# NGoetz/NF

Measured on NVIDIA B200. Metric: nis_flow_fwd_logdet_points_per_sec, higher is better.
Workload: dtype f32

## Files before the change

### nf_b200/csrc/flow_tc_h.cu

```cuda
#include <stdlib.h>
#include <cuda_fp16.h>
#include "common.cuh"
#include "spline.cuh"
#include "flow_fwd_common.cuh"
#include "tc_common.cuh"
#include "tc_spline.cuh"

#define H_SA 8.0f
#define H_AMAX 65504.0f
#define H_HID_BYTES (2 * TCH * TCH * 2)
#define H_MAXG 4
template <int KIND> struct HK {
    static constexpr int OUT_N = KIND == NIS_KIND_PWLIN ? 64 : 80;
    static constexpr int TPER = KIND == NIS_KIND_PWLIN ? 2 : 1;
    static constexpr int SLOT = KIND == NIS_KIND_PWLIN ? 32 : 80;
    static constexpr int COLS = KIND == NIS_KIND_PWLIN ? 128 : 160;
    static constexpr int COL_AHI = KIND == NIS_KIND_PWLIN ? 64 : 96;
    static constexpr int COL_ALO = COL_AHI + 32;
    static constexpr int MAXG = KIND == NIS_KIND_PWLIN ? 4 : 3;
};
__host__ __device__ static inline int h_slot(const DevFlow& F) { return F.kind == NIS_KIND_PWLIN ? 32 : 80; }
__host__ __device__ static inline int h_out_rows(const DevFlow& F) {
    int mt = 1;
    for (int c = 0; c < F.n_cells; ++c) mt = F.cells[c].T > mt ? F.cells[c].T : mt;
    const int r = mt * h_slot(F);
    return F.kind == NIS_KIND_PWLIN ? (r < 128 ? 128 : r) : r;
}
__host__ __device__ static inline int h_out_bytes(const DevFlow& F) { return 2 * h_out_rows(F) * TCH * 2; }

__host__ __device__ static inline int h_off(int row, int k) {
    return (row >> 3) * 1024 + (row & 7) * 128 + ((((k >> 3) ^ (row & 7)) << 4) | ((k & 7) << 1));
}
__host__ __device__ constexpr uint32_t h_idesc(int M, int N) {
    return (1u << 4) | ((uint32_t)(N >> 3) << 17) | ((uint32_t)(M >> 4) << 24);
}
__host__ __device__ static inline size_t h_l0_off(const DevFlow& F) { return (size_t)(F.depth - 1) * H_HID_BYTES + h_out_bytes(F); }
__host__ __device__ static inline size_t h_cell_bytes(const DevFlow& F) { return h_l0_off(F) + H_HID_BYTES + 64; }

__device__ __forceinline__ float ex2_approx(float x) {
    float y;
    asm("ex2.approx.ftz.f32 %0, %1;" : "=f"(y) : "f"(x));
    return y;
}

__device__ __forceinline__ uint32_t h_pack_sat(float x, float y) {
    uint32_t d;
    asm("cvt.rn.satfinite.f16x2.f32 %0, %1, %2;" : "=r"(d) : "f"(y), "f"(x));
    return d;
}

__device__ __forceinline__ void h_mma_ts(uint32_t tmem_d, uint32_t tmem_a, uint64_t desc_b, uint32_t idesc, uint32_t accumulate) {
    asm volatile(
        "{\n\t.reg .pred p;\n\tsetp.ne.b32 p, %4, 0;\n\t"
        "tcgen05.mma.cta_group::1.kind::f16 [%0], [%1], %2, %3, p;\n\t}"
        ::"r"(tmem_d), "r"(tmem_a), "l"(desc_b), "r"(idesc), "r"(accumulate) : "memory");
}

__global__ void __launch_bounds__(256) flow_h_pack_kernel(DevFlow F, const float* __restrict__ params, char* __restrict__ hpack) {
    __shared__ float red[8];
    __shared__ float sw_s;
    const int c = blockIdx.y, li = blockIdx.x, tid = threadIdx.x;
    const DevCell& q = F.cells[c];
    const bool outl = li == F.depth - 1, first = li == F.depth;
    const int l = first ? 0 : li + 1;
    const float* w = params + q.param_off + F.p_lin(c, l);
    const int kin = first ? q.P : TCH;
    const int rows_src = outl ? q.T * F.K : TCH, rows = outl ? h_out_rows(F) : TCH, slot = h_slot(F);
    float m = 0.f;
    for (int i = tid; i < rows_src * kin; i += 256) m = fmaxf(m, fabsf(w[i]));
#pragma unroll
    for (int o = 16; o > 0; o >>= 1) m = fmaxf(m, __shfl_xor_sync(0xffffffffu, m, o));
    if ((tid & 31) == 0) red[tid >> 5] = m;
    __syncthreads();
    if (tid == 0) {
        for (int i = 1; i < 8; ++i) m = fmaxf(m, red[i]);
        int e = 14;
        if (m > 0.f && m < 3.0e38f) frexpf(m, &e);
        e = e < -100 ? -100 : (e > 100 ? 100 : e);
        sw_s = ldexpf(1.f, 14 - e);
    }
    __syncthreads();
    const float SW = sw_s;
    char* dst = hpack + (size_t)c * h_cell_bytes(F);
    char* hi = dst + (first ? h_l0_off(F) : (size_t)li * H_HID_BYTES);
    char* lo = hi + (size_t)rows * TCH * 2;
    for (int i = tid; i < rows * TCH; i += 256) {
        const int n = i / TCH, k = i - n * TCH;
        const int t = outl ? n / slot : 0, jj = outl ? n - t * slot : n;
        const bool live = outl ? (t < q.T && jj < F.K) : k < kin;
        const float v = live ? w[(size_t)(outl ? t * F.K + jj : n) * kin + k] * SW : 0.f;
        const __half h = __float2half_rn(v);
        const int o = h_off(n, k);
        *reinterpret_cast<__half*>(hi + o) = h;
        *reinterpret_cast<__half*>(lo + o) = __float2half_rn(v - __half2float(h));
    }
    if (tid == 0) reinterpret_cast<float*>(dst + h_cell_bytes(F) - 64)[l] = 1.f / (H_SA * SW);
}

struct HSmem {
    int w0, aff, bias, st, sst, red, zb, total;
    int wfirst;
    __host__ __device__ int wl(int l) const { return (l - wfirst) * H_HID_BYTES; }
};
__host__ __device__ static inline HSmem h_layout(const DevFlow& F, int P, int l_begin, int l_end, bool zstage, int NG,
                                                 bool layer0 = true, bool stats = true) {
    HSmem s;
    int o = 0;
    s.wfirst = l_begin > 1 ? l_begin : 1;
    for (int l = s.wfirst; l <= l_end; ++l) o += l == F.depth ? h_out_bytes(F) : H_HID_BYTES;
    (void)P;
    s.w0 = o; o += layer0 ? H_HID_BYTES : 0;
    s.aff = o; o += (F.depth + 1) * 2 * TCH * 4;
    s.bias = o; o += h_out_rows(F) * 4;
    s.st = o; o += NG * (F.d + 1) * TCM * 4;
    o = (o + 15) & ~15;
    s.sst = o; o += NG * (F.d + 1) * TCM * 4;
    o = (o + 7) & ~7;
    s.red = o; o += stats ? (NG * TCM * 2 + 2 * F.maxW) * 8 : 0;
    o = (o + 127) & ~127;
    s.zb = o;
    if (zstage) o += NG * TCH * TCM * 4;
    s.total = o;
    return s;
}

__device__ __forceinline__ void h_store_act32(const float* v, const float* sc, const float* sh, uint32_t t_hi, uint32_t t_lo) {
    uint32_t hi[16], lo[16];
#pragma unroll
    for (int j4 = 0; j4 < 8; ++j4) {
        const float4 s4 = reinterpret_cast<const float4*>(sc)[j4], h4 = reinterpret_cast<const float4*>(sh)[j4];
        const float a0 = fmaxf(fmaf(v[4 * j4], s4.x, h4.x), 0.f), a1 = fmaxf(fmaf(v[4 * j4 + 1], s4.y, h4.y), 0.f);
        const float a2 = fmaxf(fmaf(v[4 * j4 + 2], s4.z, h4.z), 0.f), a3 = fmaxf(fmaf(v[4 * j4 + 3], s4.w, h4.w), 0.f);
        const uint32_t p01 = h_pack_sat(a0, a1), p23 = h_pack_sat(a2, a3);
        const float2 f01 = __half22float2(*reinterpret_cast<const __half2*>(&p01));
        const float2 f23 = __half22float2(*reinterpret_cast<const __half2*>(&p23));
        hi[2 * j4] = p01;
        hi[2 * j4 + 1] = p23;
        lo[2 * j4] = h_pack_sat(a0 - f01.x, a1 - f01.y);
        lo[2 * j4 + 1] = h_pack_sat(a2 - f23.x, a3 - f23.y);
    }
    tc_st16(t_hi, hi);
    tc_st16(t_lo, lo);
}

__device__ __forceinline__ void h_issue_block(uint32_t tmem_d, uint32_t t_hi, uint32_t t_lo, uint32_t w_hi, uint32_t w_lo, uint32_t idesc) {
#pragma unroll
    for (int ks = 0; ks < 4; ++ks) {
        h_mma_ts(tmem_d, t_hi + ks * 8, tc_desc(w_lo + ks * 32), idesc, ks > 0);
        h_mma_ts(tmem_d, t_lo + ks * 8, tc_desc(w_hi + ks * 32), idesc, 1);
    }
#pragma unroll
    for (int ks = 0; ks < 4; ++ks) h_mma_ts(tmem_d, t_hi + ks * 8, tc_desc(w_hi + ks * 32), idesc, 1);
}

template <int NG, int KIND, int MODE>
__global__ void __launch_bounds__(NG * TCM, 1) flow_cell_h_kernel(const __grid_constant__ DevFlow F, const FwdArgs A,
                                                                        const char* __restrict__ hpack) {
    constexpr int NT = NG * TCM;
    typedef HK<KIND> K_;
    constexpr int H_COLS = K_::COLS, H_COL_AHI = K_::COL_AHI, H_COL_ALO = K_::COL_ALO;
    extern __shared__ char smraw[];
    __shared__ uint64_t a_ready[NG], d_ready[NG], z_full[NG], s_full[NG];
    __shared__ uint32_t tmem_base_s;
    char* sm = smem_align1024(smraw);
    const int tid = threadIdx.x, warp = tid >> 5, lane = tid & 31;
    const int c = A.c_begin;
    const DevCell& q = F.cells[c];
    const int d = F.d, depth = F.depth;
    constexpr bool stats = (MODE & 1) != 0;
    constexpr bool from_z = (MODE & 2) != 0;
    constexpr bool nextmom = (MODE & 4) != 0;
    constexpr bool needs_state = !(from_z && stats);
    constexpr int MOM_N = 4 + 4 * 5 / 2;
    float macc[nextmom ? MOM_N : 1];
#pragma unroll
    for (int i = 0; i < (nextmom ? MOM_N : 1); ++i) macc[i] = 0.f;
    const int lz = from_z ? (A.zin_layer > 0 ? A.zin_layer : (stats ? A.stats_layer - 1 : depth)) : 1;
    const int l_end = stats ? A.stats_layer - 1 : depth;
    const bool zst = from_z || stats;
    const HSmem L = h_layout(F, q.P, lz, l_end, zst, NG, !from_z, stats);
    float* affs = reinterpret_cast<float*>(sm + L.aff);
    float* biass = reinterpret_cast<float*>(sm + L.bias);
    const float* pk = A.wpack + q.pk_off;
    const char* cellpack = hpack + (size_t)c * h_cell_bytes(F);
    const float* inv_scale = reinterpret_cast<const float*>(cellpack + h_cell_bytes(F) - 64);

    for (int l = L.wfirst; l <= l_end; ++l) {
        const int n16 = (l == depth ? h_out_bytes(F) : H_HID_BYTES) / 16;
        const uint4* src = reinterpret_cast<const uint4*>(cellpack + (size_t)(l - 1) * H_HID_BYTES);
        uint4* dst = reinterpret_cast<uint4*>(sm + L.wl(l));
        for (int i = tid; i < n16; i += NT) dst[i] = src[i];
    }
    if (!from_z) {
        const uint4* src = reinterpret_cast<const uint4*>(cellpack + h_l0_off(F));
        uint4* dst = reinterpret_cast<uint4*>(sm + L.w0);
        for (int i = tid; i < H_HID_BYTES / 16; i += NT) dst[i] = src[i];
    }
    for (int l = 0; l <= depth; ++l) {
        const int W = l == 0 ? q.P : TCH, Wp = pad8(W);
        const float* s = pk + q.aff_off[l];
        const float f = H_SA;
        const float fs = (l >= 1 && l >= lz && l <= l_end) ? f * inv_scale[l - 1] : f;
        for (int i = tid; i < W; i += NT) { affs[l * 2 * TCH + i] = fs * s[i]; affs[l * 2 * TCH + TCH + i] = f * s[Wp + i]; }
    }
    const int out_rows = h_out_rows(F);
    constexpr float LOGIT_UNIT = 1.4426950408889634f;
    for (int i = tid; i < out_rows; i += NT) {
        const int t = i / K_::SLOT, jj = i - t * K_::SLOT;
        biass[i] = (t < q.T && jj < F.K) ? LOGIT_UNIT * pk[q.bo_off + t * F.Kpad + jj] : 0.f;
    }
    if (tid == 0) {
        for (int g = 0; g < NG; ++g) {
            mbar_init(&a_ready[g], TCM); mbar_init(&d_ready[g], 1); mbar_init(&z_full[g], 1); mbar_init(&s_full[g], 1);
        }
        asm volatile("fence.mbarrier_init.release.cluster;" ::: "memory");
    }
    if (warp == 0) {
        asm volatile("tcgen05.alloc.cta_group::1.sync.aligned.shared::cta.b32 [%0], %1;" ::"r"(smem_u32(&tmem_base_s)), "r"(512));
        asm volatile("tcgen05.relinquish_alloc_permit.cta_group::1.sync.aligned;" ::);
    }
    proxy_fence();
    tc_fence_before();
    __syncthreads();
    tc_fence_after();
    const uint32_t tmem_base = tmem_base_s;
    const long long ntiles = (A.B + TCM - 1) / TCM;
    const long long rowlen = d + 1;
    const int nblk = (q.T + K_::TPER - 1) / K_::TPER;
    const bool has_out = l_end == depth;
    double dsum = 0.0, dsq = 0.0;

    const uint32_t idesc = h_idesc(TCM, TCH), idesc_out = h_idesc(TCM, K_::OUT_N);
    {
        const int g = warp >> 2, gt = tid & (TCM - 1);
        float* st = reinterpret_cast<float*>(sm + L.st) + g * (d + 1) * TCM + gt;
        const uint32_t tg = tmem_base + g * H_COLS + ((uint32_t)((warp & 3) * 32) << 16);
        uint32_t pd = 0, pa = 0, zph = 0, sph = 0;
        float* zs = reinterpret_cast<float*>(sm + L.zb) + g * TCH * TCM;
        constexpr uint32_t ZBYTES = TCH * TCM * 4;
        float* sst = reinterpret_cast<float*>(sm + L.sst) + g * (d + 1) * TCM;
        const uint32_t SBYTES = (uint32_t)((d + 1) * TCM * 4);
        const bool st_bulk = needs_state && A.from_state && (reinterpret_cast<uintptr_t>(A.state_in) & 15) == 0 && (SBYTES & 15) == 0;
        if (st_bulk && gt == 0) {
            const long long t0 = (long long)blockIdx.x * NG + g;
            if ((t0 + 1) * TCM <= A.B) bulk_load(sst, A.state_in + t0 * TCM * rowlen, SBYTES, &s_full[g]);
        }
        const float inv_out = has_out ? LOGIT_UNIT * inv_scale[depth] : 0.f;
        for (long long it = 0;; ++it) {
            const long long tile = ((long long)blockIdx.x + it * gridDim.x) * NG + g;
            if (tile >= ntiles) break;
            const long long tn = tile + (long long)gridDim.x * NG;
            if (from_z && gt == 0) {
                if (A.zout) bulk_store_wait_read();
                bulk_load(zs, A.zin + (size_t)tile * TCH * TCM, ZBYTES, &z_full[g]);
                if (tn < ntiles) bulk_prefetch_l2(A.zin + (size_t)tn * TCH * TCM, ZBYTES);
            }
            const long long pt = tile * TCM + gt;
            const bool valid = pt < A.B;
            if (!needs_state) {
            } else if (st_bulk && (tile + 1) * TCM <= A.B) {
                mbar_wait(&s_full[g], sph);
                sph ^= 1;
                for (int i = 0; i <= d; ++i) st[i * TCM] = sst[gt * rowlen + i];
                proxy_fence();
                group_sync(g);
                if (gt == 0 && (tn + 1) * TCM <= A.B) bulk_load(sst, A.state_in + tn * TCM * rowlen, SBYTES, &s_full[g]);
            } else if (valid) {
                if (A.from_state) {
                    for (int i = 0; i <= d; ++i) st[i * TCM] = A.state_in[pt * rowlen + i];
                } else {
                    for (int i = 0; i < d; ++i) st[i * TCM] = load_io(A.in, A.in_dtype, pt * A.in_cols + i);
                    st[d * TCM] = A.in_cols > d ? load_io(A.in, A.in_dtype, pt * A.in_cols + d) : 1.f;
                }
                if (!stats && A.saved && !A.from_state) {
                    float* sv = A.saved + ((long long)c * A.B + pt) * rowlen;
                    for (int i = 0; i <= d; ++i) sv[i] = st[i * TCM];
                }
            } else {
                for (int i = 0; i < d; ++i) st[i * TCM] = 0.5f;
                st[d * TCM] = 1.f;
            }
            if (from_z) { mbar_wait(&z_full[g], zph); zph ^= 1; }
            if (!from_z) {
                uint32_t hi[8], lo[8];
#pragma unroll
                for (int j2 = 0; j2 < 8; ++j2) {
                    float a0 = 0.f, a1 = 0.f;
                    if (2 * j2 < q.P) a0 = fmaf(st[q.feed[2 * j2] * TCM], affs[2 * j2], affs[TCH + 2 * j2]);
                    if (2 * j2 + 1 < q.P) a1 = fmaf(st[q.feed[2 * j2 + 1] * TCM], affs[2 * j2 + 1], affs[TCH + 2 * j2 + 1]);
                    const uint32_t p01 = h_pack_sat(a0, a1);
                    const float2 f01 = __half22float2(*reinterpret_cast<const __half2*>(&p01));
                    hi[j2] = p01;
                    lo[j2] = h_pack_sat(a0 - f01.x, a1 - f01.y);
                }
                tc_st8(tg + H_COL_AHI, hi);
                tc_st8(tg + H_COL_ALO, lo);
                tc_st_wait();
                tc_fence_before();
                mbar_arrive(&a_ready[g]);
                if (gt == 0) {
                    mbar_wait(&a_ready[g], pa);
                    tc_fence_after();
                    const uint32_t whi = smem_u32(sm + L.w0), wlo = whi + TCH * TCH * 2;
                    const uint32_t tb = tmem_base + g * H_COLS;
                    h_mma_ts(tb, tb + H_COL_AHI, tc_desc(wlo), idesc, 0);
                    h_mma_ts(tb, tb + H_COL_ALO, tc_desc(whi), idesc, 1);
                    h_mma_ts(tb, tb + H_COL_AHI, tc_desc(whi), idesc, 1);
                    tc_commit(&d_ready[g]);
                }
                pa ^= 1;
                mbar_wait(&d_ready[g], pd);
                pd ^= 1;
                tc_fence_after();
            }
            for (int l = lz; l <= l_end; ++l) {
                const float* sc = affs + l * 2 * TCH;
#pragma unroll 1
                for (int h = 0; h < 2; ++h) {
                    float v[32];
                    if (l > lz || !from_z) {
                        tc_ld32(tg + 32 * h, v);
                        tc_ld_wait();
                    } else {
                        const float* zr = zs + (32 * h) * TCM + gt;
#pragma unroll
                        for (int j = 0; j < 32; ++j) v[j] = zr[j * TCM];
                    }
                    h_store_act32(v, sc + 32 * h, sc + TCH + 32 * h, tg + H_COL_AHI + 16 * h, tg + H_COL_ALO + 16 * h);
                }
                if (l == lz && from_z) proxy_fence();
                tc_st_wait();
                tc_fence_before();
                mbar_arrive(&a_ready[g]);
                if (gt == 0) {
                    mbar_wait(&a_ready[g], pa);
                    tc_fence_after();
                    const uint32_t whi = smem_u32(sm + L.wl(l));
                    const uint32_t tb = tmem_base + g * H_COLS;
                    h_issue_block(tb, tb + H_COL_AHI, tb + H_COL_ALO, whi, whi + (l == depth ? out_rows : TCH) * TCH * 2,
                                  l == depth ? idesc_out : idesc);
                    tc_commit(&d_ready[g]);
                }
                pa ^= 1;
                if (l < depth) {
                    mbar_wait(&d_ready[g], pd);
                    pd ^= 1;
                    tc_fence_after();
                }
            }
            if (stats) {
                if (!from_z) {
                    if (gt == 0) bulk_store_wait_read();
                    group_sync(g);
                }
                const bool full = (tile + 1) * TCM <= A.B;
#pragma unroll 1
                for (int h = 0; h < 2; ++h) {
                    float v[32];
                    tc_ld32(tg + 32 * h, v);
                    tc_ld_wait();
                    if (full) {
#pragma unroll
                        for (int j = 0; j < 32; ++j) zs[(32 * h + j) * TCM + gt] = v[j];
                    } else {
#pragma unroll
                        for (int j = 0; j < 32; ++j) zs[(32 * h + j) * TCM + gt] = valid ? v[j] : 0.f;
                    }
                }
                proxy_fence();
                group_sync(g);
                if (gt == 0 && A.zout) bulk_store(A.zout + (size_t)tile * TCH * TCM, zs, ZBYTES);
                if (!A.no_stats) {
                    const float4* row = reinterpret_cast<const float4*>(zs + (gt & 63) * TCM + (gt >> 6) * 64);
                    float s_ = 0.f, q_ = 0.f;
#pragma unroll
                    for (int i = 0; i < 16; ++i) {
                        const float4 x = row[(i + lane) & 15];
                        s_ += (x.x + x.y) + (x.z + x.w);
                        q_ = fmaf(x.x, x.x, fmaf(x.y, x.y, fmaf(x.z, x.z, fmaf(x.w, x.w, q_))));
                    }
                    dsum += (double)s_; dsq += (double)q_;
                }
                proxy_fence();
                group_sync(g);
                continue;
            }
            float jfac = 1.f;
            for (int b = 0; b < nblk; ++b) {
                mbar_wait(&d_ready[g], pd);
                pd ^= 1;
                tc_fence_after();
                float z[K_::OUT_N];
                tc_ld32(tg, z);
                tc_ld32(tg + 32, z + 32);
                if (KIND != NIS_KIND_PWLIN) tc_ld16(tg + 64, z + 64);
                tc_ld_wait();
                if (b + 1 < nblk) {
                    tc_fence_before();
                    mbar_arrive(&a_ready[g]);
                    if (gt == 0) {
                        mbar_wait(&a_ready[g], pa);
                        tc_fence_after();
                        const uint32_t whi = smem_u32(sm + L.wl(depth)) + (uint32_t)(b + 1) * (K_::OUT_N * 128);
                        const uint32_t tb = tmem_base + g * H_COLS;
                        h_issue_block(tb, tb + H_COL_AHI, tb + H_COL_ALO, whi, whi + out_rows * TCH * 2, idesc_out);
                        tc_commit(&d_ready[g]);
                    }
                    pa ^= 1;
                }
                if (KIND == NIS_KIND_PWLIN) {
#pragma unroll
                    for (int tt = 0; tt < 2; ++tt) {
                        const int t = 2 * b + tt;
                        if (t >= q.T) break;
                        const float xv = st[q.trafo[t] * TCM];
                        const float a = xv * 32.f;
                        int kb = (int)floorf(a);
                        kb = kb < 0 ? 0 : (kb > 31 ? 31 : kb);
                        const float alpha = a - (float)kb;
                        const float* bs = biass + t * 32;
                        float m = -3.0e38f;
#pragma unroll
                        for (int j = 0; j < 32; ++j) { z[32 * tt + j] = fmaf(z[32 * tt + j], inv_out, bs[j]); m = fmaxf(m, z[32 * tt + j]); }
                        float e[32], s1[16], s2[8], s4[4];
#pragma unroll
                        for (int j = 0; j < 32; ++j) e[j] = ex2_approx(z[32 * tt + j] - m);
#pragma unroll
                        for (int j = 0; j < 16; ++j) s1[j] = e[2 * j] + e[2 * j + 1];
#pragma unroll
                        for (int j = 0; j < 8; ++j) s2[j] = s1[2 * j] + s1[2 * j + 1];
#pragma unroll
                        for (int j = 0; j < 4; ++j) s4[j] = s2[2 * j] + s2[2 * j + 1];
                        const float s8a = s4[0] + s4[1], s8b = s4[2] + s4[3];
                        const float S = s8a + s8b;
                        const bool b4 = kb & 16, b3 = kb & 8, b2 = kb & 4, b1 = kb & 2, b0 = kb & 1;
                        float C = b4 ? s8a : 0.f;
#pragma unroll
                        for (int j = 0; j < 16; ++j) e[j] = b4 ? e[16 + j] : e[j];
#pragma unroll
                        for (int j = 0; j < 8; ++j) s1[j] = b4 ? s1[8 + j] : s1[j];
#pragma unroll
                        for (int j = 0; j < 4; ++j) s2[j] = b4 ? s2[4 + j] : s2[j];
#pragma unroll
                        for (int j = 0; j < 2; ++j) s4[j] = b4 ? s4[2 + j] : s4[j];
                        C += b3 ? s4[0] : 0.f;
#pragma unroll
                        for (int j = 0; j < 8; ++j) e[j] = b3 ? e[8 + j] : e[j];
#pragma unroll
                        for (int j = 0; j < 4; ++j) s1[j] = b3 ? s1[4 + j] : s1[j];
#pragma unroll
                        for (int j = 0; j < 2; ++j) s2[j] = b3 ? s2[2 + j] : s2[j];
                        C += b2 ? s2[0] : 0.f;
#pragma unroll
                        for (int j = 0; j < 4; ++j) e[j] = b2 ? e[4 + j] : e[j];
#pragma unroll
                        for (int j = 0; j < 2; ++j) s1[j] = b2 ? s1[2 + j] : s1[j];
                        C += b1 ? s1[0] : 0.f;
                        const float e0 = b1 ? e[2] : e[0], e1 = b1 ? e[3] : e[1];
                        C += b0 ? e0 : 0.f;
                        const float ek = b0 ? e1 : e0;
                        const float inv = 1.f / S;
                        st[q.trafo[t] * TCM] = (ek * alpha + C) * inv;
                        jfac *= ek * inv * 32.f;
                        if (A.bins && valid) A.bins[((long long)c * A.B + pt) * d + t] = kb;
                    }
                } else {
                    const float xv = st[q.trafo[b] * TCM];
                    const float* bs = biass + b * K_::SLOT;
#pragma unroll
                    for (int j = 0; j < 65; ++j) z[j] = fmaf(z[j], inv_out, bs[j]);
                    float y, f;
                    int kb;
                    pwquad32_tree<true>(z, xv, y, f, kb);
                    st[q.trafo[b] * TCM] = y;
                    jfac *= f;
                    if (A.bins && valid) A.bins[((long long)c * A.B + pt) * d + b] = kb;
                }
            }
            st[d * TCM] *= jfac;
            if (nextmom && valid) {
                const DevCell& qn = F.cells[c + 1];
                float x[4];
#pragma unroll
                for (int k = 0; k < 4; ++k) x[k] = k < qn.P ? st[qn.feed[k] * TCM] : 0.f;
                int o = 4;
#pragma unroll
                for (int k = 0; k < 4; ++k) {
                    macc[k] += x[k];
#pragma unroll
                    for (int k2 = k; k2 < 4; ++k2) { macc[o] = fmaf(x[k], x[k2], macc[o]); ++o; }
                }
            }
            if (valid) {
                if (A.state_out) {
                    float* so = A.state_out + pt * rowlen;
                    for (int i = 0; i <= d; ++i) so[i] = st[i * TCM];
                }
                if (A.to_out) {
                    for (int i = 0; i < d; ++i) store_io(A.out, A.out_dtype, pt * rowlen + i, st[F.out_perm[i] * TCM]);
                    store_io(A.out, A.out_dtype, pt * rowlen + d, st[d * TCM]);
                }
            }
        }
    }
    bulk_store_wait_read();
    tc_fence_before();
    __syncthreads();
    if (warp == 0) asm volatile("tcgen05.dealloc.cta_group::1.sync.aligned.b32 %0, %1;" ::"r"(tmem_base), "r"(512));
    if (nextmom) {
        __shared__ bool s_last_m;
        __shared__ double sc0s_m[4 + 16];
        double* redm = reinterpret_cast<double*>(sm + L.zb);
        double* totm = redm + (NT / 32) * MOM_N;
#pragma unroll
        for (int i = 0; i < MOM_N; ++i) {
            double a = (double)macc[i];
#pragma unroll
            for (int o = 16; o > 0; o >>= 1) a += __shfl_xor_sync(0xffffffffu, a, o);
            if (lane == 0) redm[warp * MOM_N + i] = a;
        }
        __syncthreads();
        if (tid < MOM_N) {
            double s_ = 0.0;
            for (int w = 0; w < NT / 32; ++w) s_ += redm[w * MOM_N + tid];
            A.partials[(size_t)blockIdx.x * MOM_N + tid] = s_;
        }
        __threadfence();
        __syncthreads();
        if (tid == 0) s_last_m = atomicAdd(A.counter, 1u) == gridDim.x - 1;
        __syncthreads();
        if (!s_last_m) return;
        __threadfence();
        fold_partials<MOM_N>(A.partials, gridDim.x, totm + MOM_N, totm, tid, NT);
        moments_finalize<4>(F, A, c + 1, totm, sc0s_m, tid, NT);
        if (tid == 0) *A.counter = 0u;
        return;
    }
    if (!stats || A.no_stats) return;
    double* red = reinterpret_cast<double*>(sm + L.red);
    double* sacc = red + NG * TCM * 2;
    red[tid] = dsum; red[NG * TCM + tid] = dsq;
    for (int i = tid; i < 2 * F.maxW; i += NT) sacc[i] = 0.0;
    __syncthreads();
    if (tid < TCH) {
        double s = 0.0, s2 = 0.0;
        for (int k = 0; k < 2 * NG; ++k) { s += red[tid + 64 * k]; s2 += red[NG * TCM + tid + 64 * k]; }
        const double k1 = (double)inv_scale[l_end];
        sacc[tid] = s * k1; sacc[F.maxW + tid] = s2 * k1 * k1;
    }
    bn_stats_finalize(F, A, sacc, NT, red);
}

size_t nis_h_pack_floats(const DevFlow& F) {
    if (F.depth < 1) return 0;
    return (size_t)F.n_cells * (h_cell_bytes(F) / 4);
}

int64_t nis_tc_min_batch(int64_t dflt);

static int h_groups(const DevFlow& F) {
    const size_t lim = 226 * 1024;
    for (int ng = F.kind == NIS_KIND_PWLIN ? HK<NIS_KIND_PWLIN>::MAXG : HK<NIS_KIND_PWQUAD>::MAXG; ng >= 2; --ng) {
        bool ok = true;
        for (int c = 0; c < F.n_cells && ok; ++c) {
            const int P = F.cells[c].P;
            ok = (size_t)h_layout(F, P, 1, F.depth, false, ng).total + 1024 <= lim
                 && (size_t)h_layout(F, P, F.depth - 1, F.depth - 1, true, ng).total + 1024 <= lim
                 && (size_t)h_layout(F, P, F.depth, F.depth, true, ng, false, false).total + 1024 <= lim
                 && (F.depth < 3 || (size_t)h_layout(F, P, F.depth - 1, F.depth, true, ng, false, false).total + 1024 <= lim);
        }
        if (ok) return ng;
    }
    return 0;
}

bool nis_h_supported(const DevFlow& F, int64_t B, int bn_mode) {
    (void)bn_mode;
    const char* off = getenv("NIS_TC_H");
    if (off && off[0] == '0') return false;
    const char* tcoff = getenv("NIS_TC");
    if (tcoff && tcoff[0] == '0') return false;
    if (F.nb != 32 || F.depth < 1 || F.maxW != TCH) return false;
    if (F.kind == NIS_KIND_PWLIN ? F.K != 32 : F.K != 65) return false;
    if (B < nis_tc_min_batch(256)) return false;
    for (int l = 0; l < F.depth; ++l) if (F.widths[l] != TCH) return false;
    for (int c = 0; c < F.n_cells; ++c)
        if (F.cells[c].P > 16 || (F.kind == NIS_KIND_PWLIN && F.cells[c].T * 32 > 128)) return false;
    return h_groups(F) >= 2;
}

int nis_h_pack(const DevFlow& F, const float* params, float* tcpack, cudaStream_t s) {
    flow_h_pack_kernel<<<dim3(F.depth + 1, F.n_cells), 256, 0, s>>>(F, params, reinterpret_cast<char*>(tcpack));
    NIS_CUDA_CHECK_LAUNCH();
    return NIS_OK;
}

template <int NG, int KIND, int MODE>
static int h_launch_mode(const DevFlow& F, const FwdArgs& A, const char* hpack, size_t smem, int sms, cudaStream_t s) {
    static int attr_smem = 0;
    if ((int)smem > attr_smem) {
        if (cudaFuncSetAttribute(flow_cell_h_kernel<NG, KIND, MODE>, cudaFuncAttributeMaxDynamicSharedMemorySize, (int)smem) != cudaSuccess)
            return NIS_ECUDA;
        attr_smem = (int)smem;
    }
    const long long nsets = ((A.B + TCM - 1) / TCM + NG - 1) / NG;
    const int grid = (int)(nsets < sms ? nsets : sms);
    flow_cell_h_kernel<NG, KIND, MODE><<<grid, NG * TCM, smem, s>>>(F, A, hpack);
    NIS_CUDA_CHECK_LAUNCH();
    return NIS_OK;
}

template <int NG, int KIND>
static int h_launch(const DevFlow& F, const FwdArgs& A, const char* hpack, size_t smem, int sms, cudaStream_t s) {
    switch ((A.stats_layer >= 1 ? 1 : 0) | (A.zin != nullptr ? 2 : 0)) {
        case 0: return h_launch_mode<NG, KIND, 0>(F, A, hpack, smem, sms, s);
        case 1: return h_launch_mode<NG, KIND, 1>(F, A, hpack, smem, sms, s);
        case 2: return A.next_moments ? h_launch_mode<NG, KIND, 6>(F, A, hpack, smem, sms, s)
                                      : h_launch_mode<NG, KIND, 2>(F, A, hpack, smem, sms, s);
    }
    return h_launch_mode<NG, KIND, 3>(F, A, hpack, smem, sms, s);
}

int nis_launch_h(const DevFlow& F, const FwdArgs& A, const float* tcpack, cudaStream_t s) {
    static int sms = 0;
    if (sms <= 0) {
        int dev = 0;
        cudaGetDevice(&dev);
        cudaDeviceGetAttribute(&sms, cudaDevAttrMultiProcessorCount, dev);
        if (sms <= 0) sms = 148;
    }
    const bool stats = A.stats_layer >= 1;
    const int lz = A.zin ? (A.zin_layer > 0 ? A.zin_layer : (stats ? A.stats_layer - 1 : F.depth)) : 1;
    const int l_end = stats ? A.stats_layer - 1 : F.depth;
    const int ng = h_groups(F);
    const size_t smem = (size_t)h_layout(F, F.cells[A.c_begin].P, lz, l_end, A.zin != nullptr || stats, ng, A.zin == nullptr, stats).total + 1024;
    const char* hp = reinterpret_cast<const char*>(tcpack);
    if (F.kind == NIS_KIND_PWLIN) {
        switch (ng) {
            case 4: return h_launch<4, NIS_KIND_PWLIN>(F, A, hp, smem, sms, s);
            case 3: return h_launch<3, NIS_KIND_PWLIN>(F, A, hp, smem, sms, s);
            case 2: return h_launch<2, NIS_KIND_PWLIN>(F, A, hp, smem, sms, s);
        }
    } else {
        switch (ng) {
            case 3: return h_launch<3, NIS_KIND_PWQUAD>(F, A, hp, smem, sms, s);
            case 2: return h_launch<2, NIS_KIND_PWQUAD>(F, A, hp, smem, sms, s);
        }
    }
    return NIS_EUNSUPPORTED;
}
```

Before: 594.6 million.

## Add warp-specialized split kernel for final PWLIN layers with double-buffered z tiles

Adds a dedicated final-layer kernel for the piecewise-linear coupling path. Warps are split into MMA/activation warps and spline warps that communicate through TMEM and mbarriers, so the spline evaluation of one tile can overlap the tensor-core matmuls of the next. Incoming z tiles are double-buffered with bulk loads, and shared helper functions are factored out of the existing kernel. This adds barrier complexity and more shared memory, and it is gated by an environment variable and shape conditions.

```diff
diff --git a/nf_b200/csrc/flow_tc_h.cu b/nf_b200/csrc/flow_tc_h.cu
--- a/nf_b200/csrc/flow_tc_h.cu
+++ b/nf_b200/csrc/flow_tc_h.cu
@@ -103,7 +103,7 @@
     __host__ __device__ int wl(int l) const { return (l - wfirst) * H_HID_BYTES; }
 };
 __host__ __device__ static inline HSmem h_layout(const DevFlow& F, int P, int l_begin, int l_end, bool zstage, int NG,
-                                                 bool layer0 = true, bool stats = true) {
+                                                 bool layer0 = true, bool stats = true, int ztiles = 1) {
     HSmem s;
     int o = 0;
     s.wfirst = l_begin > 1 ? l_begin : 1;
@@ -119,7 +119,7 @@
     s.red = o; o += stats ? (NG * TCM * 2 + 2 * F.maxW) * 8 : 0;
     o = (o + 127) & ~127;
     s.zb = o;
-    if (zstage) o += NG * TCH * TCM * 4;
+    if (zstage) o += NG * ztiles * TCH * TCM * 4;
     s.total = o;
     return s;
 }
@@ -151,6 +151,183 @@
     }
 #pragma unroll
     for (int ks = 0; ks < 4; ++ks) h_mma_ts(tmem_d, t_hi + ks * 8, tc_desc(w_hi + ks * 32), idesc, 1);
+}
+
+constexpr float LOGIT_UNIT = 1.4426950408889634f;
+constexpr int H_MOM_N = 4 + 4 * 5 / 2;
+
+template <int KIND>
+__device__ __forceinline__ void h_stage(const DevFlow& F, const FwdArgs& A, const HSmem& L, char* sm, const char* cellpack,
+                                        int lz, int l_end, bool from_z, int tid, int NT) {
+    const DevCell& q = F.cells[A.c_begin];
+    const int depth = F.depth;
+    const float* pk = A.wpack + q.pk_off;
+    const float* inv_scale = reinterpret_cast<const float*>(cellpack + h_cell_bytes(F) - 64);
+    float* affs = reinterpret_cast<float*>(sm + L.aff);
+    float* biass = reinterpret_cast<float*>(sm + L.bias);
+    for (int l = L.wfirst; l <= l_end; ++l) {
+        const int n16 = (l == depth ? h_out_bytes(F) : H_HID_BYTES) / 16;
+        const uint4* src = reinterpret_cast<const uint4*>(cellpack + (size_t)(l - 1) * H_HID_BYTES);
+        uint4* dst = reinterpret_cast<uint4*>(sm + L.wl(l));
+        for (int i = tid; i < n16; i += NT) dst[i] = src[i];
+    }
+    if (!from_z) {
+        const uint4* src = reinterpret_cast<const uint4*>(cellpack + h_l0_off(F));
+        uint4* dst = reinterpret_cast<uint4*>(sm + L.w0);
+        for (int i = tid; i < H_HID_BYTES / 16; i += NT) dst[i] = src[i];
+    }
+    for (int l = 0; l <= depth; ++l) {
+        const int W = l == 0 ? q.P : TCH, Wp = pad8(W);
+        const float* s = pk + q.aff_off[l];
+        const float f = H_SA;
+        const float fs = (l >= 1 && l >= lz && l <= l_end) ? f * inv_scale[l - 1] : f;
+        for (int i = tid; i < W; i += NT) { affs[l * 2 * TCH + i] = fs * s[i]; affs[l * 2 * TCH + TCH + i] = f * s[Wp + i]; }
+    }
+    const int out_rows = h_out_rows(F);
+    for (int i = tid; i < out_rows; i += NT) {
+        const int t = i / HK<KIND>::SLOT, jj = i - t * HK<KIND>::SLOT;
+        biass[i] = (t < q.T && jj < F.K) ? LOGIT_UNIT * pk[q.bo_off + t * F.Kpad + jj] : 0.f;
+    }
+}
+
+__device__ __forceinline__ void h_load_state(const DevFlow& F, const FwdArgs& A, int c, float* st, float* sst, uint64_t* s_full,
+                                             uint32_t& sph, bool st_bulk, long long tile, long long tn, int gt, int bar, bool save) {
+    const int d = F.d;
+    const long long rowlen = d + 1, pt = tile * TCM + gt;
+    if (st_bulk && (tile + 1) * TCM <= A.B) {
+        mbar_wait(s_full, sph);
+        sph ^= 1;
+        for (int i = 0; i <= d; ++i) st[i * TCM] = sst[gt * rowlen + i];
+        proxy_fence();
+        group_sync(bar);
+        if (gt == 0 && (tn + 1) * TCM <= A.B) bulk_load(sst, A.state_in + tn * TCM * rowlen, (uint32_t)(rowlen * TCM * 4), s_full);
+    } else if (pt < A.B) {
+        if (A.from_state) {
+            for (int i = 0; i <= d; ++i) st[i * TCM] = A.state_in[pt * rowlen + i];
+        } else {
+            for (int i = 0; i < d; ++i) st[i * TCM] = load_io(A.in, A.in_dtype, pt * A.in_cols + i);
+            st[d * TCM] = A.in_cols > d ? load_io(A.in, A.in_dtype, pt * A.in_cols + d) : 1.f;
+        }
+        if (save && A.saved && !A.from_state) {
+            float* sv = A.saved + ((long long)c * A.B + pt) * rowlen;
+            for (int i = 0; i <= d; ++i) sv[i] = st[i * TCM];
+        }
+    } else {
+        for (int i = 0; i < d; ++i) st[i * TCM] = 0.5f;
+        st[d * TCM] = 1.f;
+    }
+}
+
+__device__ __forceinline__ void h_pwlin32(float* z, float xv, float inv_out, const float* bs, float& y, float& f, int& kb) {
+    const float a = xv * 32.f;
+    kb = (int)floorf(a);
+    kb = kb < 0 ? 0 : (kb > 31 ? 31 : kb);
+    const float alpha = a - (float)kb;
+    float m = -3.0e38f;
+#pragma unroll
+    for (int j = 0; j < 32; ++j) { z[j] = fmaf(z[j], inv_out, bs[j]); m = fmaxf(m, z[j]); }
+    float e[32], s1[16], s2[8], s4[4];
+#pragma unroll
+    for (int j = 0; j < 32; ++j) e[j] = ex2_approx(z[j] - m);
+#pragma unroll
+    for (int j = 0; j < 16; ++j) s1[j] = e[2 * j] + e[2 * j + 1];
+#pragma unroll
+    for (int j = 0; j < 8; ++j) s2[j] = s1[2 * j] + s1[2 * j + 1];
+#pragma unroll
+    for (int j = 0; j < 4; ++j) s4[j] = s2[2 * j] + s2[2 * j + 1];
+    const float s8a = s4[0] + s4[1], s8b = s4[2] + s4[3];
+    const float S = s8a + s8b;
+    const bool b4 = kb & 16, b3 = kb & 8, b2 = kb & 4, b1 = kb & 2, b0 = kb & 1;
+    float C = b4 ? s8a : 0.f;
+#pragma unroll
+    for (int j = 0; j < 16; ++j) e[j] = b4 ? e[16 + j] : e[j];
+#pragma unroll
+    for (int j = 0; j < 8; ++j) s1[j] = b4 ? s1[8 + j] : s1[j];
+#pragma unroll
+    for (int j = 0; j < 4; ++j) s2[j] = b4 ? s2[4 + j] : s2[j];
+#pragma unroll
+    for (int j = 0; j < 2; ++j) s4[j] = b4 ? s4[2 + j] : s4[j];
+    C += b3 ? s4[0] : 0.f;
+#pragma unroll
+    for (int j = 0; j < 8; ++j) e[j] = b3 ? e[8 + j] : e[j];
+#pragma unroll
+    for (int j = 0; j < 4; ++j) s1[j] = b3 ? s1[4 + j] : s1[j];
+#pragma unroll
+    for (int j = 0; j < 2; ++j) s2[j] = b3 ? s2[2 + j] : s2[j];
+    C += b2 ? s2[0] : 0.f;
+#pragma unroll
+    for (int j = 0; j < 4; ++j) e[j] = b2 ? e[4 + j] : e[j];
+#pragma unroll
+    for (int j = 0; j < 2; ++j) s1[j] = b2 ? s1[2 + j] : s1[j];
+    C += b1 ? s1[0] : 0.f;
+    const float e0 = b1 ? e[2] : e[0], e1 = b1 ? e[3] : e[1];
+    C += b0 ? e0 : 0.f;
+    const float ek = b0 ? e1 : e0;
+    const float inv = 1.f / S;
+    y = (ek * alpha + C) * inv;
+    f = ek * inv * 32.f;
+}
+
+template <bool NEXTMOM>
+__device__ __forceinline__ void h_point_out(const DevFlow& F, const FwdArgs& A, int c, const float* st, long long pt, bool valid,
+                                            float* macc) {
+    const int d = F.d;
+    if (NEXTMOM && valid) {
+        const DevCell& qn = F.cells[c + 1];
+        float x[4];
+#pragma unroll
+        for (int k = 0; k < 4; ++k) x[k] = k < qn.P ? st[qn.feed[k] * TCM] : 0.f;
+        int o = 4;
+#pragma unroll
+        for (int k = 0; k < 4; ++k) {
+            macc[k] += x[k];
+#pragma unroll
+            for (int k2 = k; k2 < 4; ++k2) { macc[o] = fmaf(x[k], x[k2], macc[o]); ++o; }
+        }
+    }
+    if (valid) {
+        const long long rowlen = d + 1;
+        if (A.state_out) {
+            float* so = A.state_out + pt * rowlen;
+            for (int i = 0; i <= d; ++i) so[i] = st[i * TCM];
+        }
+        if (A.to_out) {
+            for (int i = 0; i < d; ++i) store_io(A.out, A.out_dtype, pt * rowlen + i, st[F.out_perm[i] * TCM]);
+            store_io(A.out, A.out_dtype, pt * rowlen + d, st[d * TCM]);
+        }
+    }
+}
+
+__device__ __forceinline__ void h_warp_moments(const float* macc, double* row, int lane) {
+#pragma unroll
+    for (int i = 0; i < H_MOM_N; ++i) {
+        double a = (double)macc[i];
+#pragma unroll
+        for (int o = 16; o > 0; o >>= 1) a += __shfl_xor_sync(0xffffffffu, a, o);
+        if (lane == 0) row[i] = a;
+    }
+}
+
+template <int NT, int NW>
+__device__ __forceinline__ void h_fold_next_moments(const DevFlow& F, const FwdArgs& A, int c, double* redm, int tid) {
+    __shared__ bool s_last_m;
+    __shared__ double sc0s_m[4 + 16];
+    double* totm = redm + NW * H_MOM_N;
+    __syncthreads();
+    if (tid < H_MOM_N) {
+        double s_ = 0.0;
+        for (int w = 0; w < NW; ++w) s_ += redm[w * H_MOM_N + tid];
+        A.partials[(size_t)blockIdx.x * H_MOM_N + tid] = s_;
+    }
+    __threadfence();
+    __syncthreads();
+    if (tid == 0) s_last_m = atomicAdd(A.counter, 1u) == gridDim.x - 1;
+    __syncthreads();
+    if (!s_last_m) return;
+    __threadfence();
+    fold_partials<H_MOM_N>(A.partials, gridDim.x, totm + H_MOM_N, totm, tid, NT);
+    moments_finalize<4>(F, A, c + 1, totm, sc0s_m, tid, NT);
+    if (tid == 0) *A.counter = 0u;
 }
 
 template <int NG, int KIND, int MODE>
@@ -171,44 +348,20 @@
     constexpr bool from_z = (MODE & 2) != 0;
     constexpr bool nextmom = (MODE & 4) != 0;
     constexpr bool needs_state = !(from_z && stats);
-    constexpr int MOM_N = 4 + 4 * 5 / 2;
-    float macc[nextmom ? MOM_N : 1];
-#pragma unroll
-    for (int i = 0; i < (nextmom ? MOM_N : 1); ++i) macc[i] = 0.f;
+    float macc[nextmom ? H_MOM_N : 1];
+#pragma unroll
+    for (int i = 0; i < (nextmom ? H_MOM_N : 1); ++i) macc[i] = 0.f;
     const int lz = from_z ? (A.zin_layer > 0 ? A.zin_layer : (stats ? A.stats_layer - 1 : depth)) : 1;
     const int l_end = stats ? A.stats_layer - 1 : depth;
     const bool zst = from_z || stats;
     const HSmem L = h_layout(F, q.P, lz, l_end, zst, NG, !from_z, stats);
-    float* affs = reinterpret_cast<float*>(sm + L.aff);
-    float* biass = reinterpret_cast<float*>(sm + L.bias);
-    const float* pk = A.wpack + q.pk_off;
+    const float* affs = reinterpret_cast<const float*>(sm + L.aff);
+    const float* biass = reinterpret_cast<const float*>(sm + L.bias);
     const char* cellpack = hpack + (size_t)c * h_cell_bytes(F);
     const float* inv_scale = reinterpret_cast<const float*>(cellpack + h_cell_bytes(F) - 64);
 
-    for (int l = L.wfirst; l <= l_end; ++l) {
-        const int n16 = (l == depth ? h_out_bytes(F) : H_HID_BYTES) / 16;
-        const uint4* src = reinterpret_cast<const uint4*>(cellpack + (size_t)(l - 1) * H_HID_BYTES);
-        uint4* dst = reinterpret_cast<uint4*>(sm + L.wl(l));
-        for (int i = tid; i < n16; i += NT) dst[i] = src[i];
-    }
-    if (!from_z) {
-        const uint4* src = reinterpret_cast<const uint4*>(cellpack + h_l0_off(F));
-        uint4* dst = reinterpret_cast<uint4*>(sm + L.w0);
-        for (int i = tid; i < H_HID_BYTES / 16; i += NT) dst[i] = src[i];
-    }
-    for (int l = 0; l <= depth; ++l) {
-        const int W = l == 0 ? q.P : TCH, Wp = pad8(W);
-        const float* s = pk + q.aff_off[l];
-        const float f = H_SA;
-        const float fs = (l >= 1 && l >= lz && l <= l_end) ? f * inv_scale[l - 1] : f;
-        for (int i = tid; i < W; i += NT) { affs[l * 2 * TCH + i] = fs * s[i]; affs[l * 2 * TCH + TCH + i] = f * s[Wp + i]; }
-    }
+    h_stage<KIND>(F, A, L, sm, cellpack, lz, l_end, from_z, tid, NT);
     const int out_rows = h_out_rows(F);
-    constexpr float LOGIT_UNIT = 1.4426950408889634f;
-    for (int i = tid; i < out_rows; i += NT) {
-        const int t = i / K_::SLOT, jj = i - t * K_::SLOT;
-        biass[i] = (t < q.T && jj < F.K) ? LOGIT_UNIT * pk[q.bo_off + t * F.Kpad + jj] : 0.f;
-    }
     if (tid == 0) {
         for (int g = 0; g < NG; ++g) {
             mbar_init(&a_ready[g], TCM); mbar_init(&d_ready[g], 1); mbar_init(&z_full[g], 1); mbar_init(&s_full[g], 1);
@@ -257,29 +410,7 @@
             }
             const long long pt = tile * TCM + gt;
             const bool valid = pt < A.B;
-            if (!needs_state) {
-            } else if (st_bulk && (tile + 1) * TCM <= A.B) {
-                mbar_wait(&s_full[g], sph);
-                sph ^= 1;
-                for (int i = 0; i <= d; ++i) st[i * TCM] = sst[gt * rowlen + i];
-                proxy_fence();
-                group_sync(g);
-                if (gt == 0 && (tn + 1) * TCM <= A.B) bulk_load(sst, A.state_in + tn * TCM * rowlen, SBYTES, &s_full[g]);
-            } else if (valid) {
-                if (A.from_state) {
-                    for (int i = 0; i <= d; ++i) st[i * TCM] = A.state_in[pt * rowlen + i];
-                } else {
-                    for (int i = 0; i < d; ++i) st[i * TCM] = load_io(A.in, A.in_dtype, pt * A.in_cols + i);
-                    st[d * TCM] = A.in_cols > d ? load_io(A.in, A.in_dtype, pt * A.in_cols + d) : 1.f;
-                }
-                if (!stats && A.saved && !A.from_state) {
-                    float* sv = A.saved + ((long long)c * A.B + pt) * rowlen;
-                    for (int i = 0; i <= d; ++i) sv[i] = st[i * TCM];
-                }
-            } else {
-                for (int i = 0; i < d; ++i) st[i * TCM] = 0.5f;
-                st[d * TCM] = 1.f;
-            }
+            if (needs_state) h_load_state(F, A, c, st, sst, &s_full[g], sph, st_bulk, tile, tn, gt, g, !stats);
             if (from_z) { mbar_wait(&z_full[g], zph); zph ^= 1; }
             if (!from_z) {
                 uint32_t hi[8], lo[8];
@@ -413,55 +544,11 @@
                     for (int tt = 0; tt < 2; ++tt) {
                         const int t = 2 * b + tt;
                         if (t >= q.T) break;
-                        const float xv = st[q.trafo[t] * TCM];
-                        const float a = xv * 32.f;
-                        int kb = (int)floorf(a);
-                        kb = kb < 0 ? 0 : (kb > 31 ? 31 : kb);
-                        const float alpha = a - (float)kb;
-                        const float* bs = biass + t * 32;
-                        float m = -3.0e38f;
-#pragma unroll
-                        for (int j = 0; j < 32; ++j) { z[32 * tt + j] = fmaf(z[32 * tt + j], inv_out, bs[j]); m = fmaxf(m, z[32 * tt + j]); }
-                        float e[32], s1[16], s2[8], s4[4];
-#pragma unroll
-                        for (int j = 0; j < 32; ++j) e[j] = ex2_approx(z[32 * tt + j] - m);
-#pragma unroll
-                        for (int j = 0; j < 16; ++j) s1[j] = e[2 * j] + e[2 * j + 1];
-#pragma unroll
-                        for (int j = 0; j < 8; ++j) s2[j] = s1[2 * j] + s1[2 * j + 1];
-#pragma unroll
-                        for (int j = 0; j < 4; ++j) s4[j] = s2[2 * j] + s2[2 * j + 1];
-                        const float s8a = s4[0] + s4[1], s8b = s4[2] + s4[3];
-                        const float S = s8a + s8b;
-                        const bool b4 = kb & 16, b3 = kb & 8, b2 = kb & 4, b1 = kb & 2, b0 = kb & 1;
-                        float C = b4 ? s8a : 0.f;
-#pragma unroll
-                        for (int j = 0; j < 16; ++j) e[j] = b4 ? e[16 + j] : e[j];
-#pragma unroll
-                        for (int j = 0; j < 8; ++j) s1[j] = b4 ? s1[8 + j] : s1[j];
-#pragma unroll
-                        for (int j = 0; j < 4; ++j) s2[j] = b4 ? s2[4 + j] : s2[j];
-#pragma unroll
-                        for (int j = 0; j < 2; ++j) s4[j] = b4 ? s4[2 + j] : s4[j];
-                        C += b3 ? s4[0] : 0.f;
-#pragma unroll
-                        for (int j = 0; j < 8; ++j) e[j] = b3 ? e[8 + j] : e[j];
-#pragma unroll
-                        for (int j = 0; j < 4; ++j) s1[j] = b3 ? s1[4 + j] : s1[j];
-#pragma unroll
-                        for (int j = 0; j < 2; ++j) s2[j] = b3 ? s2[2 + j] : s2[j];
-                        C += b2 ? s2[0] : 0.f;
-#pragma unroll
-                        for (int j = 0; j < 4; ++j) e[j] = b2 ? e[4 + j] : e[j];
-#pragma unroll
-                        for (int j = 0; j < 2; ++j) s1[j] = b2 ? s1[2 + j] : s1[j];
-                        C += b1 ? s1[0] : 0.f;
-                        const float e0 = b1 ? e[2] : e[0], e1 = b1 ? e[3] : e[1];
-                        C += b0 ? e0 : 0.f;
-                        const float ek = b0 ? e1 : e0;
-                        const float inv = 1.f / S;
-                        st[q.trafo[t] * TCM] = (ek * alpha + C) * inv;
-                        jfac *= ek * inv * 32.f;
+                        float y, f;
+                        int kb;
+                        h_pwlin32(z + 32 * tt, st[q.trafo[t] * TCM], inv_out, biass + t * 32, y, f, kb);
+                        st[q.trafo[t] * TCM] = y;
+                        jfac *= f;
                         if (A.bins && valid) A.bins[((long long)c * A.B + pt) * d + t] = kb;
                     }
                 } else {
@@ -478,29 +565,7 @@
                 }
             }
             st[d * TCM] *= jfac;
-            if (nextmom && valid) {
-                const DevCell& qn = F.cells[c + 1];
-                float x[4];
-#pragma unroll
-                for (int k = 0; k < 4; ++k) x[k] = k < qn.P ? st[qn.feed[k] * TCM] : 0.f;
-                int o = 4;
-#pragma unroll
-                for (int k = 0; k < 4; ++k) {
-                    macc[k] += x[k];
-#pragma unroll
-                    for (int k2 = k; k2 < 4; ++k2) { macc[o] = fmaf(x[k], x[k2], macc[o]); ++o; }
-                }
-            }
-            if (valid) {
-                if (A.state_out) {
-                    float* so = A.state_out + pt * rowlen;
-                    for (int i = 0; i <= d; ++i) so[i] = st[i * TCM];
-                }
-                if (A.to_out) {
-                    for (int i = 0; i < d; ++i) store_io(A.out, A.out_dtype, pt * rowlen + i, st[F.out_perm[i] * TCM]);
-                    store_io(A.out, A.out_dtype, pt * rowlen + d, st[d * TCM]);
-                }
-            }
+            h_point_out<nextmom>(F, A, c, st, pt, valid, macc);
         }
     }
     bulk_store_wait_read();
@@ -508,32 +573,9 @@
     __syncthreads();
     if (warp == 0) asm volatile("tcgen05.dealloc.cta_group::1.sync.aligned.b32 %0, %1;" ::"r"(tmem_base), "r"(512));
     if (nextmom) {
-        __shared__ bool s_last_m;
-        __shared__ double sc0s_m[4 + 16];
         double* redm = reinterpret_cast<double*>(sm + L.zb);
-        double* totm = redm + (NT / 32) * MOM_N;
-#pragma unroll
-        for (int i = 0; i < MOM_N; ++i) {
-            double a = (double)macc[i];
-#pragma unroll
-            for (int o = 16; o > 0; o >>= 1) a += __shfl_xor_sync(0xffffffffu, a, o);
-            if (lane == 0) redm[warp * MOM_N + i] = a;
-        }
-        __syncthreads();
-        if (tid < MOM_N) {
-            double s_ = 0.0;
-            for (int w = 0; w < NT / 32; ++w) s_ += redm[w * MOM_N + tid];
-            A.partials[(size_t)blockIdx.x * MOM_N + tid] = s_;
-        }
-        __threadfence();
-        __syncthreads();
-        if (tid == 0) s_last_m = atomicAdd(A.counter, 1u) == gridDim.x - 1;
-        __syncthreads();
-        if (!s_last_m) return;
-        __threadfence();
-        fold_partials<MOM_N>(A.partials, gridDim.x, totm + MOM_N, totm, tid, NT);
-        moments_finalize<4>(F, A, c + 1, totm, sc0s_m, tid, NT);
-        if (tid == 0) *A.counter = 0u;
+        h_warp_moments(macc, redm + warp * H_MOM_N, lane);
+        h_fold_next_moments<NT, NT / 32>(F, A, c, redm, tid);
         return;
     }
     if (!stats || A.no_stats) return;
@@ -549,6 +591,181 @@
         sacc[tid] = s * k1; sacc[F.maxW + tid] = s2 * k1 * k1;
     }
     bn_stats_finalize(F, A, sacc, NT, red);
+}
+
+#define HS_PAIRS 2
+#define HS_GROUPS 4
+#define HS_COL_AHI 64
+#define HS_COL_ALO 96
+#define HS_COL_L 128
+template <bool NEXTMOM>
+__global__ void __launch_bounds__(HS_PAIRS * 2 * TCM, 1) flow_final_h_split_kernel(const __grid_constant__ DevFlow F, const FwdArgs A,
+                                                                                   const char* __restrict__ hpack) {
+    constexpr int NT = HS_PAIRS * 2 * TCM;
+    extern __shared__ char smraw[];
+    __shared__ uint64_t z_full[HS_PAIRS][2], s_full[HS_PAIRS], a_ready[HS_PAIRS], d_ready[HS_PAIRS], out_done[HS_PAIRS],
+        l_full[HS_PAIRS], l_empty[HS_PAIRS];
+    __shared__ uint32_t tmem_base_s;
+    char* sm = smem_align1024(smraw);
+    const int tid = threadIdx.x, warp = tid >> 5;
+    const int c = A.c_begin;
+    const DevCell& q = F.cells[c];
+    const int d = F.d, depth = F.depth;
+    const int lz = A.zin_layer > 0 ? A.zin_layer : depth;
+    const HSmem L = h_layout(F, q.P, lz, depth, true, HS_PAIRS, false, false, 2);
+    const char* cellpack = hpack + (size_t)c * h_cell_bytes(F);
+    const float* inv_scale = reinterpret_cast<const float*>(cellpack + h_cell_bytes(F) - 64);
+    const float* affs = reinterpret_cast<const float*>(sm + L.aff);
+    const float* biass = reinterpret_cast<const float*>(sm + L.bias);
+    h_stage<NIS_KIND_PWLIN>(F, A, L, sm, cellpack, lz, depth, true, tid, NT);
+    if (tid == 0) {
+        for (int p = 0; p < HS_PAIRS; ++p) {
+            mbar_init(&z_full[p][0], 1); mbar_init(&z_full[p][1], 1); mbar_init(&s_full[p], 1);
+            mbar_init(&a_ready[p], TCM); mbar_init(&d_ready[p], 1); mbar_init(&out_done[p], 1);
+            mbar_init(&l_full[p], 1); mbar_init(&l_empty[p], TCM);
+        }
+        asm volatile("fence.mbarrier_init.release.cluster;" ::: "memory");
+    }
+    if (warp == 0) {
+        asm volatile("tcgen05.alloc.cta_group::1.sync.aligned.shared::cta.b32 [%0], %1;" ::"r"(smem_u32(&tmem_base_s)), "r"(512));
+        asm volatile("tcgen05.relinquish_alloc_permit.cta_group::1.sync.aligned;" ::);
+    }
+    proxy_fence();
+    tc_fence_before();
+    __syncthreads();
+    tc_fence_after();
+    const uint32_t tmem_base = tmem_base_s;
+    const long long ntiles = (A.B + TCM - 1) / TCM;
+    const int p = warp >> 3, gt = tid & (TCM - 1);
+    const bool spline_role = (warp & 4) != 0;
+    const uint32_t tp = tmem_base + p * 256;
+    const uint32_t tl = tp + ((uint32_t)((warp & 3) * 32) << 16);
+    auto tile_of = [&](long long it) {
+        return ((long long)blockIdx.x + (it >> 1) * gridDim.x) * HS_GROUPS + 2 * p + (int)(it & 1);
+    };
+    float macc[NEXTMOM ? H_MOM_N : 1], macc2[NEXTMOM ? H_MOM_N : 1];
+#pragma unroll
+    for (int i = 0; i < (NEXTMOM ? H_MOM_N : 1); ++i) macc[i] = macc2[i] = 0.f;
+
+    if (!spline_role) {
+        constexpr uint32_t ZBYTES = TCH * TCM * 4;
+        float* zs = reinterpret_cast<float*>(sm + L.zb) + p * 2 * TCH * TCM;
+        if (gt == 0) {
+            for (int s = 0; s < 2; ++s)
+                if (tile_of(s) < ntiles) bulk_load(zs + s * TCH * TCM, A.zin + (size_t)tile_of(s) * TCH * TCM, ZBYTES, &z_full[p][s]);
+        }
+        const uint32_t idesc = h_idesc(TCM, TCH), idesc_out = h_idesc(TCM, 32 * q.T);
+        const int out_rows = h_out_rows(F);
+        uint32_t pa = 0, pd = 0;
+        for (long long it = 0;; ++it) {
+            const long long tile = tile_of(it);
+            if (tile >= ntiles) break;
+            const int slot = (int)(it & 1);
+            float* zsl = zs + slot * TCH * TCM;
+            mbar_wait(&z_full[p][slot], (uint32_t)(it >> 1) & 1);
+            if (it > 0) {
+                mbar_wait(&out_done[p], (uint32_t)(it - 1) & 1);
+                tc_fence_after();
+            }
+            for (int l = lz; l <= depth; ++l) {
+                const float* sc = affs + l * 2 * TCH;
+#pragma unroll 1
+                for (int h = 0; h < 2; ++h) {
+                    float v[32];
+                    if (l > lz) {
+                        tc_ld32(tl + 32 * h, v);
+                        tc_ld_wait();
+                    } else {
+                        const float* zr = zsl + (32 * h) * TCM + gt;
+#pragma unroll
+                        for (int j = 0; j < 32; ++j) v[j] = zr[j * TCM];
+                    }
+                    h_store_act32(v, sc + 32 * h, sc + TCH + 32 * h, tl + HS_COL_AHI + 16 * h, tl + HS_COL_ALO + 16 * h);
+                }
+                if (l == lz) proxy_fence();
+                tc_st_wait();
+                tc_fence_before();
+                mbar_arrive(&a_ready[p]);
+                if (gt == 0) {
+                    mbar_wait(&a_ready[p], pa);
+                    if (l == lz && tile_of(it + 2) < ntiles)
+                        bulk_load(zsl, A.zin + (size_t)tile_of(it + 2) * TCH * TCM, ZBYTES, &z_full[p][slot]);
+                    if (l == depth && it > 0) mbar_wait(&l_empty[p], (uint32_t)(it - 1) & 1);
+                    tc_fence_after();
+                    const uint32_t whi = smem_u32(sm + L.wl(l));
+                    if (l < depth) {
+                        h_issue_block(tp, tp + HS_COL_AHI, tp + HS_COL_ALO, whi, whi + TCH * TCH * 2, idesc);
+                        tc_commit(&d_ready[p]);
+                    } else {
+                        h_issue_block(tp + HS_COL_L, tp + HS_COL_AHI, tp + HS_COL_ALO, whi, whi + out_rows * TCH * 2, idesc_out);
+                        tc_commit(&out_done[p]);
+                        tc_commit(&l_full[p]);
+                    }
+                }
+                pa ^= 1;
+                if (l < depth) {
+                    mbar_wait(&d_ready[p], pd);
+                    pd ^= 1;
+                    tc_fence_after();
+                }
+            }
+        }
+    } else {
+        float* st = reinterpret_cast<float*>(sm + L.st) + p * (d + 1) * TCM + gt;
+        float* sst = reinterpret_cast<float*>(sm + L.sst) + p * (d + 1) * TCM;
+        const long long rowlen = d + 1;
+        const uint32_t SBYTES = (uint32_t)(rowlen * TCM * 4);
+        const bool st_bulk = A.from_state && (reinterpret_cast<uintptr_t>(A.state_in) & 15) == 0 && (SBYTES & 15) == 0;
+        const float inv_out = LOGIT_UNIT * inv_scale[depth];
+        if (st_bulk && gt == 0 && (tile_of(0) + 1) * TCM <= A.B) bulk_load(sst, A.state_in + tile_of(0) * TCM * rowlen, SBYTES, &s_full[p]);
+        uint32_t sph = 0;
+        long long it = 0;
+        for (;; ++it) {
+            const long long tile = tile_of(it);
+            if (tile >= ntiles) break;
+            const long long pt = tile * TCM + gt;
+            const bool valid = pt < A.B;
+            h_load_state(F, A, c, st, sst, &s_full[p], sph, st_bulk, tile, tile_of(it + 1), gt, HS_PAIRS + p, true);
+            mbar_wait(&l_full[p], (uint32_t)it & 1);
+            tc_fence_after();
+            float jfac = 1.f;
+#pragma unroll 1
+            for (int t = 0; t < q.T; ++t) {
+                float z[32];
+                tc_ld32(tl + HS_COL_L + 32 * t, z);
+                tc_ld_wait();
+                if (t == q.T - 1) {
+                    tc_fence_before();
+                    mbar_arrive(&l_empty[p]);
+                }
+                float y, f;
+                int kb;
+                h_pwlin32(z, st[q.trafo[t] * TCM], inv_out, biass + t * 32, y, f, kb);
+                st[q.trafo[t] * TCM] = y;
+                jfac *= f;
+                if (A.bins && valid) A.bins[((long long)c * A.B + pt) * d + t] = kb;
+            }
+            st[d * TCM] *= jfac;
+            h_point_out<NEXTMOM>(F, A, c, st, pt, valid, macc);
+#pragma unroll
+            for (int i = 0; i < (NEXTMOM ? H_MOM_N : 1); ++i) { const float m = macc[i]; macc[i] = macc2[i]; macc2[i] = m; }
+        }
+        if (it & 1) {
+#pragma unroll
+            for (int i = 0; i < (NEXTMOM ? H_MOM_N : 1); ++i) { const float m = macc[i]; macc[i] = macc2[i]; macc2[i] = m; }
+        }
+    }
+    tc_fence_before();
+    __syncthreads();
+    if (warp == 0) asm volatile("tcgen05.dealloc.cta_group::1.sync.aligned.b32 %0, %1;" ::"r"(tmem_base), "r"(512));
+    if (NEXTMOM) {
+        double* redm = reinterpret_cast<double*>(sm + L.zb);
+        if (spline_role) {
+            h_warp_moments(macc, redm + ((2 * p) * 4 + (warp & 3)) * H_MOM_N, tid & 31);
+            h_warp_moments(macc2, redm + ((2 * p + 1) * 4 + (warp & 3)) * H_MOM_N, tid & 31);
+        }
+        h_fold_next_moments<NT, HS_GROUPS * 4>(F, A, c, redm, tid);
+    }
 }
 
 size_t nis_h_pack_floats(const DevFlow& F) {
@@ -621,6 +838,31 @@
     return h_launch_mode<NG, KIND, 3>(F, A, hpack, smem, sms, s);
 }
 
+static size_t h_split_final_smem(const DevFlow& F, const FwdArgs& A, int lz) {
+    const char* e = getenv("NIS_H_SPLIT_FINAL");
+    if (e && e[0] == '0') return 0;
+    if (F.kind != NIS_KIND_PWLIN || !A.zin || A.zout || A.stats_layer >= 1 || lz < F.depth - 1) return 0;
+    const DevCell& q = F.cells[A.c_begin];
+    if (q.T < 1 || q.T > 4 || q.P > 16) return 0;
+    const size_t smem = (size_t)h_layout(F, q.P, lz, F.depth, true, HS_PAIRS, false, false, 2).total + 1024;
+    return smem <= 226 * 1024 ? smem : 0;
+}
+
+template <bool NEXTMOM>
+static int h_launch_split(const DevFlow& F, const FwdArgs& A, const char* hpack, size_t smem, int sms, cudaStream_t s) {
+    static int attr_smem = 0;
+    if ((int)smem > attr_smem) {
+        if (cudaFuncSetAttribute(flow_final_h_split_kernel<NEXTMOM>, cudaFuncAttributeMaxDynamicSharedMemorySize, (int)smem) != cudaSuccess)
+            return NIS_ECUDA;
+        attr_smem = (int)smem;
+    }
+    const long long nsets = ((A.B + TCM - 1) / TCM + HS_GROUPS - 1) / HS_GROUPS;
+    const int grid = (int)(nsets < sms ? nsets : sms);
+    flow_final_h_split_kernel<NEXTMOM><<<grid, HS_PAIRS * 2 * TCM, smem, s>>>(F, A, hpack);
+    NIS_CUDA_CHECK_LAUNCH();
+    return NIS_OK;
+}
+
 int nis_launch_h(const DevFlow& F, const FwdArgs& A, const float* tcpack, cudaStream_t s) {
     static int sms = 0;
     if (sms <= 0) {
@@ -632,6 +874,10 @@
     const bool stats = A.stats_layer >= 1;
     const int lz = A.zin ? (A.zin_layer > 0 ? A.zin_layer : (stats ? A.stats_layer - 1 : F.depth)) : 1;
     const int l_end = stats ? A.stats_layer - 1 : F.depth;
+    if (const size_t smem = h_split_final_smem(F, A, lz)) {
+        const char* hp = reinterpret_cast<const char*>(tcpack);
+        return A.next_moments ? h_launch_split<true>(F, A, hp, smem, sms, s) : h_launch_split<false>(F, A, hp, smem, sms, s);
+    }
     const int ng = h_groups(F);
     const size_t smem = (size_t)h_layout(F, F.cells[A.c_begin].P, lz, l_end, A.zin != nullptr || stats, ng, A.zin == nullptr, stats).total + 1024;
     const char* hp = reinterpret_cast<const char*>(tcpack);
```

Result: faster. 606.1 million, median of 6 (+1.9%).
